# limanling/clip-event

Measured on AMD Instinct MI355X. Metric: image-text pairs/sec/GPU, ViT-B/32 224px x 77-tok, global-batch contrastive, higher is better.
Workload: dtype bf16; 1 GPU; ViT-B/32 224px x 77-tok, bf16 operands, per-GPU batch 256, K=1, InfoNCE only, full train step (fwd+bwd+clip_grad_norm+Adam), random-init weights; global_batch=256, parallelism=dp1, captions=SOT + U[8,75] random ids + EOT, zero-padded to 77 (SURVEY 8(d) c2), text_rows=live tokens SOT..EOT only: 54.8% of B*77 rows (identical results, see DESIGN.md), fresh_captions_every_step=True, alignment=False, cu_hog=0, nt_pgrid=256, full=False

## Files before the change

### clip_event_amd/csrc/attention.hip

```cpp
#include <map>
#include <mutex>

#include <type_traits>

#include "common.hpp"
#include "../../include/clip_event_hip.h"

namespace {

constexpr int HD = 64;
constexpr int ROW = 160;

typedef __attribute__((address_space(3))) s16x4 lds_s16x4;
typedef __attribute__((ext_vector_type(8))) short s16x8;

__device__ __forceinline__ bf16x8 tr_pair(const char* p0, const char* p1) {
    s16x4 lo = __builtin_amdgcn_ds_read_tr16_b64_v4i16((lds_s16x4*)p0);
    s16x4 hi = __builtin_amdgcn_ds_read_tr16_b64_v4i16((lds_s16x4*)p1);
    s16x8 v = {lo[0], lo[1], lo[2], lo[3], hi[0], hi[1], hi[2], hi[3]};
    return __builtin_bit_cast(bf16x8, v);
}

__device__ __forceinline__ bf16x8 pack8(const f32x4& a, const f32x4& b) {
    u32x4 v = {pack_bf2(a[0], a[1]), pack_bf2(a[2], a[3]), pack_bf2(b[0], b[1]), pack_bf2(b[2], b[3])};
// ... 793 lines not shown
        for (int ct = 0; ct < 4; ++ct) ak[kt][ct] *= scale;
        if (jok[kt]) {
            bf16_t* krow = dbase + (long)j[kt] * lddq + D + 4 * g;
            bf16_t* vrow = dbase + (long)j[kt] * lddq + 2 * D + 4 * g;
#pragma unroll
            for (int ct = 0; ct < 4; ++ct) {
                u32x2 pk = {pack_bf2(ak[kt][ct][0], ak[kt][ct][1]), pack_bf2(ak[kt][ct][2], ak[kt][ct][3])};
                u32x2 pv = {pack_bf2(av[kt][ct][0], av[kt][ct][1]), pack_bf2(av[kt][ct][2], av[kt][ct][3])};
                *reinterpret_cast<u32x2*>(krow + ct * 16) = pk;
                *reinterpret_cast<u32x2*>(vrow + ct * 16) = pv;
            }
        }
        if (bias_grad) {
            float vk[16], vv[16];
#pragma unroll
            for (int ct = 0; ct < 4; ++ct)
#pragma unroll
                for (int r = 0; r < 4; ++r) {
                    vk[ct * 4 + r] = ak[kt][ct][r];
                    vv[ct * 4 + r] = av[kt][ct][r];
                }
            const float tk = row16_colsum(vk, li), tv = row16_colsum(vv, li);
            const int k = row16_colsum_index(li);
            atomicAdd(&csum[(k >> 2) * 16 + 4 * g + (k & 3)], tk);
            atomicAdd(&csum[64 + (k >> 2) * 16 + 4 * g + (k & 3)], tv);
        }
    }
    if (bias_grad) {
        __syncthreads();
        if (tid < 128) atomicAdd(bias_grad + (1 + (tid >> 6)) * D + h * HD + (tid & 63), csum[tid]);
    }
}

int tiles_for(int L) { return ((L + 31) / 32) * 2; }
int attn_xcd_order() {
    static const int v = getenv("CE_ATTN_XCD") ? atoi(getenv("CE_ATTN_XCD")) : 1;
    return v;
}

struct StreamScratch { float* p = nullptr; size_t cap = 0; };
std::mutex g_scratch_mu;
std::map<hipStream_t, StreamScratch> g_scratch;
float* delta_scratch(hipStream_t s, size_t floats) {
    std::lock_guard<std::mutex> lk(g_scratch_mu);
    StreamScratch& e = g_scratch[s];
    if (e.cap < floats) {
        if (e.p) hipFree(e.p);
        e.p = nullptr; e.cap = 0;
        if (hipMalloc(reinterpret_cast<void**>(&e.p), floats * sizeof(float)) != hipSuccess) return nullptr;
        e.cap = floats;
    }
    return e.p;
}

}

#define ATTN_DISPATCH(T, CALL)                 \
    switch (T) {                               \
        case 2: CALL(2); break;                \
        case 4: CALL(4); break;                \
        case 6: CALL(6); break;                \
        case 8: CALL(8); break;                \
        default: CE_CHECK_ARG(false, "attention: sequence length %d not supported", L); \
    }

extern "C" int ce_attention_fwd(const void* qkv, long ld, void* o, long ldo, float* lse, const int* cu_seqlens, int B,
// ... 61 lines not shown
        if (nk == 1)
            hipLaunchKernelGGL(attn_bwd_long_dkv_kernel<1>, grid1, dim3(256), 0, sl, (const bf16_t*)qkv, ld, (const bf16_t*)o, ldo,
                               (const bf16_t*)dout, lddo, lse, (bf16_t*)dqkv, lddq, bias_grad, delta, L, H, D, causal, 0.125f, attn_xcd_order());
        else
            hipLaunchKernelGGL(attn_bwd_long_dkv_kernel<2>, grid2, dim3(256), 0, sl, (const bf16_t*)qkv, ld, (const bf16_t*)o, ldo,
                               (const bf16_t*)dout, lddo, lse, (bf16_t*)dqkv, lddq, bias_grad, delta, L, H, D, causal, 0.125f, attn_xcd_order());
        CE_LAUNCH_CHECK();
        return 0;
    }
    const int T = tiles_for(L);
    const int Lp = T * 16;
    int nw = T;
    if (nw > 8) nw = 8;
    const size_t lds = 2 * (size_t)Lp * ROW + 2 * (size_t)Lp * (Lp * 2 + 32);
    const float scale = 0.125f;
    hipStream_t s = (hipStream_t)stream;
    CeProfScope prof(CE_PROF_ATTN_BWD, 10.0 * B * H * (double)L * L * HD, 2.0 * (double)B * L * (8.0 * D), s);
#define CALL(TT)                                                                                                   \
    do {                                                                                                           \
        static std::once_flag attr;                                                                                \
        std::call_once(attr, [] {                                                                                  \
            hipFuncSetAttribute(reinterpret_cast<const void*>(attn_bwd_kernel<TT>),                                \
                                hipFuncAttributeMaxDynamicSharedMemorySize, 160 * 1024);                           \
        });                                                                                                        \
        hipLaunchKernelGGL(attn_bwd_kernel<TT>, dim3(B * H), dim3(64 * nw), lds, s, (const bf16_t*)qkv, ld,        \
                           (const bf16_t*)o, ldo, (const bf16_t*)dout, lddo, lse, (bf16_t*)dqkv, lddq, bias_grad, cu_seqlens, L, \
                           H, D, causal, scale);                                                                           \
    } while (0)
    ATTN_DISPATCH(T, CALL);
#undef CALL
    CE_LAUNCH_CHECK();
    return 0;
}
```

### clip_event_amd/csrc/gemm.hip

```cpp
#include <stdlib.h>

#include <map>
#include <mutex>
#include <type_traits>

#include "common.hpp"
#include "nt_plan.hpp"
#include "../../include/clip_event_hip.h"

#ifndef CE_DIAG_TN3
#define CE_DIAG_TN3 0
#endif

namespace {

constexpr int NT_BM = 128, NT_BN = 128, NT_BK = 64;
constexpr int NT_STAGE_BYTES = (NT_BM + NT_BN) * NT_BK * 2;
constexpr int NT_LDS_BYTES = 2 * NT_STAGE_BYTES;

#include "gemm_common.hpp"

template <int EPI>
__global__ __launch_bounds__(256, 2) void gemm_nt_kernel(NTArgs p) {
    extern __shared__ __attribute__((aligned(16))) char smem[];
// ... 1364 lines not shown
            const char* st = smem + cur * T2_STAGE_BYTES;
#pragma unroll
            for (int s = 0; s < 4; ++s) {
                bf16x8 pf[2], qf[2];
#pragma unroll
                for (int t = 0; t < 2; ++t) {
                    pf[t] = tr_frag2(st + offP[t] + s * 16 * 256);
                    qf[t] = tr_frag2(st + offQ[t] + s * 16 * 256);
                }
#pragma unroll
                for (int nt = 0; nt < 2; ++nt)
#pragma unroll
                    for (int kt = 0; kt < 2; ++kt)
                        acc[nt][kt] = __builtin_amdgcn_mfma_f32_32x32x16_bf16(pf[nt], qf[kt], acc[nt][kt], 0, 0, 0);
            }
            asm volatile("s_waitcnt vmcnt(0)" ::: "memory");
            __syncthreads();
        }

        const int ek = k0 + wk * 64 + (lane & 31);
        const int en = n0 + wn * 64 + 4 * (lane >> 5);
        constexpr bool sole = false;
#pragma unroll
        for (int nt = 0; nt < 2; ++nt)
#pragma unroll
            for (int kt = 0; kt < 2; ++kt) {
                const int k = ek + kt * 32;
                if (k >= p.Kk) continue;
#pragma unroll
                for (int r = 0; r < 16; ++r) {
                    const int n = en + nt * 32 + (r & 3) + 8 * (r >> 2);
                    if (n < p.Nn) {
                        float* o = p.out + (long)n * p.ldo + k;
                        if (sole) *o += acc[nt][kt][r];
                        else atomicAdd(o, acc[nt][kt][r]);
                    }
                }
            }
    }
}

template <int T3_ROWS, int T3_STAGES>
__global__ __launch_bounds__(1024, 4) void gemm_tn3_kernel(TNGroup grp) {
    constexpr int T3_IMG_BYTES = T3_ROWS * 256;
    constexpr int T3_STAGE_BYTES = 4 * T3_IMG_BYTES;
    constexpr int KSTEPS = T3_ROWS / 16;
    constexpr int DPW = T3_ROWS / 16;
    extern __shared__ __attribute__((aligned(16))) char smem[];
    const int tid = threadIdx.x;
    const int lane = tid & 63;
    const int wave = __builtin_amdgcn_readfirstlane(tid >> 6);
    const int wn = wave >> 2, wk = wave & 3;

    const int m_tiles = (grp.M + TN_BM - 1) / TN_BM;
    const int mps = grp.m_per_split / TN_BM;
    const int s_r = lane >> 4;
    const int s_chunk = (lane & 15) ^ (s_r << 2);
    const int g = lane >> 4, li = lane & 15;
    const int t_row = 8 * (g >> 1) + (li >> 2);
    const int t_sw = (li >> 2) << 2;
    const int t_cb = 2 * (g & 1) + ((li & 3) >> 1);
    int offP[2], offQ[2];
#pragma unroll
    for (int t = 0; t < 2; ++t) {
        offP[t] = (wn >> 1) * T3_IMG_BYTES + t_row * 256 + ((((wn & 1) * 8 + t * 4 + t_cb) ^ t_sw) << 4) + (li & 1) * 8;
        offQ[t] = (2 + (wk >> 1)) * T3_IMG_BYTES + t_row * 256 + ((((wk & 1) * 8 + t * 4 + t_cb) ^ t_sw) << 4) + (li & 1) * 8;
    }
// ... 586 lines not shown
            const long tail = wgs - (rounds - 1) * 256;
            return rounds * (ce_div_up(m_tiles, sp) * 1.7 + 3.0) + tail * (sp == 1 ? 0.105 : 0.20);
        };
        int sp = 1;
        if (splits > 0) sp = splits;
        else if (force_splits > 0) sp = force_splits;
        else {
            double best = cost(1);
            for (int c = 2; c <= 16 && c <= m_tiles && (long)tiles3 * c <= 256; ++c)
                if (cost(c) < best) { best = cost(c); sp = c; }
        }
        if (sp > m_tiles) sp = m_tiles;
        if (sp < 1) sp = 1;
        g.m_per_split = ce_div_up(m_tiles, sp) * TN_BM;
        g.splits = ce_div_up(M, g.m_per_split);
        g.overwrite = (overwrite && g.splits == 1) ? 1 : 0;
        if (overwrite && !g.overwrite && zero_outputs() != 0) return -5;
        static int depth = getenv("CE_TN3_DEPTH") ? atoi(getenv("CE_TN3_DEPTH")) : 3;
        g.depth = depth < 1 ? 1 : (depth > 3 ? 3 : depth);
        CeProfScope prof(CE_PROF_GEMM_TN, flops, bytes, s);
        static int rows48 = getenv("CE_TN3_ROWS") ? atoi(getenv("CE_TN3_ROWS")) != 32 : 1;
        static int lw = getenv("CE_TN3_LW") ? atoi(getenv("CE_TN3_LW")) : 1;
        if (lw && rows48)
            hipLaunchKernelGGL((gemm_tn3lw_kernel<48, 3>), dim3((unsigned)(tiles3 * g.splits)), dim3(768), 3 * 48 * 1024, s, g);
        else if (lw)
            hipLaunchKernelGGL((gemm_tn3lw_kernel<32, 4>), dim3((unsigned)(tiles3 * g.splits)), dim3(768), 4 * 32 * 1024, s, g);
        else if (rows48)
            hipLaunchKernelGGL((gemm_tn3_kernel<48, 3>), dim3((unsigned)(tiles3 * g.splits)), dim3(1024), 3 * 48 * 1024, s, g);
        else
            hipLaunchKernelGGL((gemm_tn3_kernel<32, 4>), dim3((unsigned)(tiles3 * g.splits)), dim3(1024), 4 * 32 * 1024, s, g);
        CE_LAUNCH_CHECK();
        return 0;
    }
    if (overwrite && zero_outputs() != 0) return -5;
    if (splits <= 0) splits = 512 / tiles;
    if (splits > m_tiles) splits = m_tiles;
    if (splits < 1) splits = 1;
    g.m_per_split = ce_div_up(m_tiles, splits) * TN_BM;
    g.splits = ce_div_up(M, g.m_per_split);
    CeProfScope prof(CE_PROF_GEMM_TN2, flops, bytes, s);
    hipLaunchKernelGGL(gemm_tn2_kernel, dim3((unsigned)(tiles * g.splits)), dim3(256), T2_LDS_BYTES, s, g);
    CE_LAUNCH_CHECK();
    return 0;
}

extern "C" int ce_probe_mfma(int shape, const void* a_frags, const void* b_frags, float* out, void* stream) {
    if (shape == 16)
        hipLaunchKernelGGL(probe_mfma16_kernel, dim3(1), dim3(64), 0, (hipStream_t)stream, (const bf16x8*)a_frags,
                           (const bf16x8*)b_frags, (f32x4*)out);
    else if (shape == 32)
        hipLaunchKernelGGL(probe_mfma32_kernel, dim3(1), dim3(64), 0, (hipStream_t)stream, (const bf16x8*)a_frags,
                           (const bf16x8*)b_frags, (f32x16*)out);
    else
        CE_CHECK_ARG(false, "ce_probe_mfma: shape must be 16 or 32");
    CE_LAUNCH_CHECK();
    return 0;
}

extern "C" int ce_probe_tr16(const void* image, int n_elems, const int* byte_off, void* out, void* stream) {
    CE_CHECK_ARG(n_elems > 0 && n_elems <= 16384, "ce_probe_tr16: image must hold 1..16384 elements");
    hipLaunchKernelGGL(probe_tr16_kernel, dim3(1), dim3(64), n_elems * 2, (hipStream_t)stream, (const uint16_t*)image,
                       n_elems, byte_off, (s16x4*)out);
    CE_LAUNCH_CHECK();
    return 0;
}
```

### clip_event_amd/csrc/tower.cpp

```cpp
#include <hip/hip_runtime.h>
#include <stdlib.h>

#include <map>
#include <mutex>

#include "common.hpp"
#include "../../include/clip_event_hip.h"

namespace {

constexpr int WG_MAX_BLOCKS = 8;
constexpr int WG_SETS = WG_MAX_BLOCKS + 1;
constexpr int LNP_RING = 8;

struct Carver {
    char* base;
    size_t off = 0;
    explicit Carver(void* b) : base(reinterpret_cast<char*>(b)) {}
    template <typename T>
    T* take(size_t n) {
        off = (off + 255) & ~size_t(255);
        T* p = base ? reinterpret_cast<T*>(base + off) : nullptr;
        off += n * sizeof(T);
        return p;
// ... 115 lines not shown

int linear(bool use8, const Layout& L, const void*& q8_of, const void* A, long lda, const void* W, const void* W8, const float* S8, int M,
           int N, int K, int epi, const float* bias, const void* resid, long ldr, void* out, long ldo, void* out2,
           long ldo2, const void* aux, long ldaux, void* stream) {
    if (use8 && W8 && S8 && K % 128 == 0 && K <= 4096) {
        if (q8_of != A || lda != K) TRY(ce_quant_rows_fp8(A, lda, L.q8, K, L.q8s, M, K, stream));
        q8_of = nullptr;
        return ce_gemm_nt_fp8(L.q8, K, L.q8s, W8, K, S8, M, N, K, epi, bias, resid, ldr, out, ldo, out2, ldo2, aux, ldaux,
                              stream);
    }
    return ce_gemm_nt(A, lda, W, K, M, N, K, epi, bias, resid, ldr, out, ldo, out2, ldo2, aux, ldaux, stream);
}

int forward_run(const ce_tower_desc* d, int batch, int rows, const int* cu_seqlens, const void* x0, Layout& L, void* x_out,
                const int* sel_rows, bool infer, void* stream) {
    const int M = rows, w = d->width;
    const bool f8 = (d->fp8 & 1) != 0;
    const int ST = d->stream16 ? CE_T_F16 : CE_T_F32;
    const int EPI_RESID = d->stream16 ? CE_EPI_BIAS_RESID_F16 : CE_EPI_BIAS_RESID_F32;
    const int EPI_FC = infer ? CE_EPI_BIAS_QGELU_BF16 : CE_EPI_BIAS_GELU;
    const long esz = d->stream16 ? 2 : 4;
    const void* x = x0;
    const void* q8_of = nullptr;
    const bool lnq = f8 && w % 128 == 0 && w <= 4096;
    for (int l = 0; l < d->layers; ++l) {
        const ce_block_params& p = d->blocks[l];
        BlockStash& s = L.blk[l];
        void* xo = (l + 1 < d->layers) ? s.x_out : x_out;
        TRY(ce_layernorm_fwd_q8(x, ST, w, nullptr, p.ln1_w, p.ln1_b, s.h1, CE_T_BF16, w, s.mean1, s.rstd1, M, w, 1e-5f,
                                lnq ? L.q8 : nullptr, w, L.q8s, stream));
        if (lnq) q8_of = s.h1;
        TRY(linear(f8, L, q8_of, s.h1, w, p.w_qkv, p.w8_qkv, p.s8_qkv, M, 3 * w, w, CE_EPI_BIAS_BF16, p.b_qkv, nullptr, 0, s.qkv, 3 * w, nullptr, 0,
                       nullptr, 0, stream));
        TRY(ce_attention_fwd(s.qkv, 3 * w, s.o, w, s.lse, cu_seqlens, batch, d->tokens, d->heads, d->causal, stream));
        if (sel_rows && l + 1 == d->layers) {
            const int Bn = batch;
            TRY(ce_copy_rows(s.o, w * 2L, sel_rows, L.os, w * 2L, nullptr, Bn, w * 2, stream));
            TRY(ce_copy_rows(x, w * esz, sel_rows, L.xs_in, w * esz, nullptr, Bn, (int)(w * esz), stream));
            TRY(linear(f8, L, q8_of, L.os, w, p.w_out, p.w8_out, p.s8_out, Bn, w, w, EPI_RESID, p.b_out, L.xs_in, w, L.xs_mid, w, nullptr,
                           0, nullptr, 0, stream));
            TRY(ce_layernorm_fwd_t(L.xs_mid, ST, w, nullptr, p.ln2_w, p.ln2_b, L.h2s, CE_T_BF16, w, L.means, L.rstds, Bn, w, 1e-5f, stream));
            TRY(linear(f8, L, q8_of, L.h2s, w, p.w_fc, p.w8_fc, p.s8_fc, Bn, 4 * w, w, EPI_FC, p.b_fc, nullptr, 0, infer ? L.gs : L.as, 4 * w,
                           infer ? nullptr : L.gs, infer ? 0 : 4 * w, nullptr, 0, stream));
            TRY(linear(f8, L, q8_of, L.gs, 4 * w, p.w_proj, p.w8_proj, p.s8_proj, Bn, w, 4 * w, EPI_RESID, p.b_proj, L.xs_mid, w, x_out, w,
                           nullptr, 0, nullptr, 0, stream));
            break;
        }
        TRY(linear(f8, L, q8_of, s.o, w, p.w_out, p.w8_out, p.s8_out, M, w, w, EPI_RESID, p.b_out, x, w, s.x_mid, w, nullptr, 0, nullptr,
                       0, stream));
        TRY(ce_layernorm_fwd_q8(s.x_mid, ST, w, nullptr, p.ln2_w, p.ln2_b, s.h2, CE_T_BF16, w, s.mean2, s.rstd2, M, w, 1e-5f,
                                lnq ? L.q8 : nullptr, w, L.q8s, stream));
        if (lnq) q8_of = s.h2;
        TRY(linear(f8, L, q8_of, s.h2, w, p.w_fc, p.w8_fc, p.s8_fc, M, 4 * w, w, EPI_FC, p.b_fc, nullptr, 0, infer ? s.g : s.a, 4 * w,
                       infer ? nullptr : s.g, infer ? 0 : 4 * w, nullptr, 0, stream));
        TRY(linear(f8, L, q8_of, s.g, 4 * w, p.w_proj, p.w8_proj, p.s8_proj, M, w, 4 * w, EPI_RESID, p.b_proj, s.x_mid, w, xo, w,
                       nullptr, 0, nullptr, 0, stream));
        x = xo;
    }
    return 0;
}

}

extern "C" size_t ce_tower_workspace_bytes(const ce_tower_desc* d, int batch) {
    if (check_desc(d, batch) != 0) return 0;
    Layout L;
    carve(d, batch, (size_t)batch * d->tokens, nullptr, L);
    return L.bytes;
}

// ... 104 lines not shown
    } pend;
    auto queue = [&](const void* P, long ldp, const void* Q, long ldq, int Nn, int Kk, float* out, long ldo) {
        const int i = pend.count++;
        pend.P[i] = P; pend.ldp[i] = ldp; pend.Q[i] = Q; pend.ldq[i] = ldq;
        pend.Nn[i] = Nn; pend.Kk[i] = Kk; pend.out[i] = out; pend.ldo[i] = ldo;
    };
    auto flush = [&]() -> int {
        if (pend.count == 0) return 0;
        const int rc = ce_gemm_tn_grouped_ex(pend.count, pend.P, pend.ldp, pend.Q, pend.ldq, M, pend.Nn, pend.Kk, pend.out,
                                             pend.ldo, 0, d->wgrad_overwrite, stream);
        pend.count = 0;
        pend.blocks = 0;
        return rc;
    };
    int top = layer_hi;
    if (layer_hi < last) {
    } else if (sel_rows) {
        CE_CHECK_ARG(dx_sel, "ce_tower_backward: pruned mode needs dx_sel");
        const int l = top, Bn = batch, q = l % WG_SETS;
        const ce_block_params& p = d->blocks[l];
        BlockStash& s = L.blk[l];
        const void* x_in = (l == 0) ? x0 : L.blk[l - 1].x_out;
        TRY(ce_cast_bf16(dx_sel, L.dxbs, (long)Bn * w, stream));
        TRY(linear(b8, L, q8_of, L.dxbs, w, p.wt_proj, p.wt8_proj, p.st8_proj, Bn, 4 * w, w, CE_EPI_GELUGRAD_BF16, nullptr, nullptr, 0, L.das, 4 * w, nullptr,
                       0, L.as, 4 * w, stream));
        TRY(ce_colsum_bf16(L.dxbs, w, p.g_b_proj, Bn, w, stream));
        TRY(linear(b8, L, q8_of, L.das, 4 * w, p.wt_fc, p.wt8_fc, p.st8_fc, Bn, w, 4 * w, CE_EPI_BF16, nullptr, nullptr, 0, L.dhs, w, nullptr, 0,
                       nullptr, 0, stream));
        TRY(ce_colsum_bf16(L.das, 4 * w, p.g_b_fc, Bn, 4 * w, stream));
        TRY(ce_layernorm_bwd_t(L.dhs, CE_T_BF16, w, L.xs_mid, ST, w, nullptr, L.means, L.rstds, p.ln2_w, dx_sel, CE_T_F32, L.dxs_mid,
                               ST, w, L.dxb2s, w, p.g_ln2_w, p.g_ln2_b, p.g_b_out, GS, Bn, w, stream));
        TRY(linear(b8, L, q8_of, L.dxb2s, w, p.wt_out, p.wt8_out, p.st8_out, Bn, w, w, CE_EPI_BF16, nullptr, nullptr, 0, L.dos, w, nullptr, 0, nullptr, 0,
                       stream));
        TRY(ce_scatter_rows_zero(L.dos, w * 2L, L.d_o, w * 2L, sel_rows, Bn, M, w * 2, stream));
        TRY(ce_attention_bwd(s.qkv, 3 * w, s.o, w, L.d_o, w, s.lse, L.dqkv[q], 3 * w, p.g_b_qkv, cu_seqlens, batch, d->tokens, d->heads,
                             d->causal, stream));
        {
            const void* P[3] = {L.dxbs, L.das, L.dxb2s};
            const long ldp[3] = {w, 4L * w, w};
            const void* Q[3] = {L.gs, L.h2s, L.os};
            const long ldq[3] = {4L * w, w, w};
            const int Nn[3] = {w, 4 * w, w};
            const int Kk[3] = {4 * w, w, w};
            float* out[3] = {p.g_w_proj, p.g_w_fc, p.g_w_out};
            const long ldo[3] = {4L * w, w, w};
            TRY(ce_gemm_tn_grouped_ex(3, P, ldp, Q, ldq, Bn, Nn, Kk, out, ldo, 0, d->wgrad_overwrite, stream));
        }
        queue(L.dqkv[q], 3L * w, s.h1, w, 3 * w, w, p.g_w_qkv, w);
        TRY(linear(b8, L, q8_of, L.dqkv[q], 3 * w, p.wt_qkv, p.wt8_qkv, p.st8_qkv, M, w, 3 * w, CE_EPI_BF16, nullptr, nullptr, 0, L.dh, w, nullptr, 0,
                       nullptr, 0, stream));
        TRY(ce_scatter_rows_zero(L.dxs_mid, w * esz, dx, w * esz, sel_rows, Bn, M, (int)(w * esz), stream));
        TRY(ce_layernorm_bwd_t(L.dh, CE_T_BF16, w, x_in, ST, w, nullptr, s.mean1, s.rstd1, p.ln1_w, dx, ST, dx, ST, w,
                               L.dxb[(l + WG_SETS - 1) % WG_SETS], w, p.g_ln1_w, p.g_ln1_b,
                               (l > 0) ? d->blocks[l - 1].g_b_proj : nullptr, GS, M, w, stream));
        top = l - 1;
    } else {
        if (d->stream16) TRY(ce_cast_scaled(dx, ST, L.dxb[top % WG_SETS], CE_T_BF16, GS, 1, (long)M * w, stream));
        else TRY(ce_cast_bf16(reinterpret_cast<const float*>(dx), L.dxb[top % WG_SETS], (long)M * w, stream));
    }
    plan_cuts(top, layer_lo, pend.count > 0 ? ((w % 256 == 0 && M >= 2048) ? 3L * (w / 256) * (w / 256)
                                                                              : 3L * ((w + 127) / 128) * ((w + 127) / 128)) : 0);
    for (int l = top; l >= layer_lo; --l) {
        const ce_block_params& p = d->blocks[l];
        BlockStash& s = L.blk[l];
        const int q = l % WG_SETS;
        bf16_t *dxb_a = L.dxb[q], *dxb_b = L.dxb2[q], *da = L.da[q], *dqkv = L.dqkv[q];
        const void* x_in = (l == 0) ? x0 : L.blk[l - 1].x_out;
        TRY(linear(b8, L, q8_of, dxb_a, w, p.wt_proj, p.wt8_proj, p.st8_proj, M, 4 * w, w, CE_EPI_GELUGRAD_BF16, nullptr, nullptr, 0, da, 4 * w, p.g_b_fc,
                       4 * w, s.a, 4 * w, stream));
// ... 27 lines not shown
```

### clip_event_amd/ops.py

```python
from __future__ import annotations

from ctypes import c_float, c_int, c_long, c_void_p
from typing import Optional

import torch

from . import _lib as L
from ._lib import check, lib, ptr, stream


def _rows(t: torch.Tensor) -> int:
    return t.shape[0]


def gemm_nt(a: torch.Tensor, b: torch.Tensor, epilogue: int, *, bias=None, resid=None, out=None, out2=None,
            aux=None, M: Optional[int] = None) -> torch.Tensor:
    assert a.dtype == torch.bfloat16 and b.dtype == torch.bfloat16 and a.is_cuda and b.is_cuda
    M = a.shape[0] if M is None else M
    K = a.shape[1]
    N = b.shape[0]
    assert b.shape[1] == K
    f32_out = epilogue in (L.EPI_F32, L.EPI_BIAS_F32, L.EPI_BIAS_RESID_F32)
    if epilogue == L.EPI_BIAS_RESID_F16:
        assert resid is not None and resid.dtype == torch.float16
# ... 61 lines not shown
def layernorm_bwd_t(dy, x, mean, rstd, w, dw, db, dx_out, *, gscale=None, rows=None, dx_in=None, dxb=None, dxsum=None):
    M, D = dy.shape
    check(lib().ce_layernorm_bwd_t(ptr(dy), c_int(_TYPE[dy.dtype]), c_long(dy.stride(0)), ptr(x), c_int(_TYPE[x.dtype]),
                                   c_long(x.stride(0)), ptr(rows), ptr(mean), ptr(rstd), ptr(w), ptr(dx_in),
                                   c_int(_TYPE[dx_in.dtype] if dx_in is not None else L.T_F32), ptr(dx_out),
                                   c_int(_TYPE[dx_out.dtype]), c_long(dx_out.stride(0)), ptr(dxb),
                                   c_long(dxb.stride(0) if dxb is not None else 0), ptr(dw), ptr(db), ptr(dxsum),
                                   ptr(gscale), c_int(M), c_int(D), stream()), "ce_layernorm_bwd_t")
    return dx_out


def grad_scale(x: torch.Tensor, target: float = 1024.0) -> torch.Tensor:
    assert x.dtype == torch.float32 and x.is_contiguous()
    buf = torch.empty(257, device=x.device, dtype=torch.float32)
    check(lib().ce_grad_scale(ptr(x), c_long(x.numel()), c_float(target), c_void_p(buf.data_ptr() + 4), ptr(buf), stream()),
          "ce_grad_scale")
    return buf[:1]


def cast_scaled(x: torch.Tensor, dtype, scale: torch.Tensor, divide: bool = False):
    y = torch.empty_like(x, dtype=dtype)
    check(lib().ce_cast_scaled(ptr(x), c_int(_TYPE[x.dtype]), ptr(y), c_int(_TYPE[dtype]), ptr(scale), c_int(1 if divide else 0),
                               c_long(x.numel()), stream()), "ce_cast_scaled")
    return y


def cast_t(x: torch.Tensor, dtype, mul: float = 1.0):
    y = torch.empty_like(x, dtype=dtype)
    check(lib().ce_cast_t(ptr(x), c_int(_TYPE[x.dtype]), ptr(y), c_int(_TYPE[dtype]), c_float(mul), c_long(x.numel()), stream()),
          "ce_cast_t")
    return y


def attention_fwd(qkv: torch.Tensor, B: int, L: int, H: int, causal: bool, cu_seqlens=None):
    assert qkv.dtype == torch.bfloat16
    o = torch.empty(qkv.shape[0], H * 64, device=qkv.device, dtype=torch.bfloat16)
    lse = torch.empty(B * H * L, device=qkv.device, dtype=torch.float32)
    check(lib().ce_attention_fwd(ptr(qkv), c_long(qkv.stride(0)), ptr(o), c_long(o.stride(0)), ptr(lse),
                                 ptr(cu_seqlens), c_int(B), c_int(L), c_int(H), c_int(1 if causal else 0), stream()),
          "ce_attention_fwd")
    return o, lse


def attention_bwd(qkv, o, dout, lse, B: int, L: int, H: int, causal: bool, bias_grad=None, cu_seqlens=None):
    dqkv = torch.empty_like(qkv)
    check(lib().ce_attention_bwd(ptr(qkv), c_long(qkv.stride(0)), ptr(o), c_long(o.stride(0)), ptr(dout),
                                 c_long(dout.stride(0)), ptr(lse), ptr(dqkv), c_long(dqkv.stride(0)), ptr(bias_grad),
                                 ptr(cu_seqlens), c_int(B), c_int(L), c_int(H), c_int(1 if causal else 0), stream()),
          "ce_attention_bwd")
    return dqkv


def probe_mfma(shape: int, a_frags: torch.Tensor, b_frags: torch.Tensor) -> torch.Tensor:
    out = torch.empty(64, 4 if shape == 16 else 16, device=a_frags.device, dtype=torch.float32)
    check(lib().ce_probe_mfma(c_int(shape), ptr(a_frags), ptr(b_frags), ptr(out), stream()), "ce_probe_mfma")
    return out


def probe_tr16(image: torch.Tensor, byte_off: torch.Tensor) -> torch.Tensor:
    out = torch.empty(64, 4, device=image.device, dtype=torch.int16)
    check(lib().ce_probe_tr16(ptr(image), c_int(image.numel()), ptr(byte_off), ptr(out), stream()), "ce_probe_tr16")
    return out


def quant_rows_fp8(x: torch.Tensor):
    assert x.dtype == torch.bfloat16 and x.is_cuda and x.stride(1) == 1
    M, K = x.shape
    q = torch.empty(M, K, dtype=torch.uint8, device=x.device)
    scale = torch.empty(M, dtype=torch.float32, device=x.device)
    check(lib().ce_quant_rows_fp8(ptr(x), c_long(x.stride(0)), ptr(q), c_long(K), ptr(scale), c_int(M), c_int(K), stream()),
          "ce_quant_rows_fp8")
    return q, scale


def gemm_nt_fp8(a8, sa, b8, sb, epilogue: int, *, bias=None, resid=None, aux=None, colsum=None):
    M, K = a8.shape
    N = b8.shape[0]
    f32_out = epilogue == L.EPI_BIAS_RESID_F32
# ... 56 lines not shown
```

### include/clip_event_hip.h

```cpp
#ifndef CLIP_EVENT_HIP_H
#define CLIP_EVENT_HIP_H

#include <stddef.h>
#include <stdint.h>

#ifdef __cplusplus
extern "C" {
#endif

const char* ce_last_error(void);
int ce_version(void);

enum {
    CE_EPI_BF16 = 0,
    CE_EPI_F32 = 1,
    CE_EPI_BIAS_BF16 = 2,
    CE_EPI_BIAS_F32 = 3,
    CE_EPI_BIAS_RESID_F32 = 4,
    CE_EPI_BIAS_GELU = 5,
    CE_EPI_GELUGRAD_BF16 = 6,
    CE_EPI_BIAS_RESID_F16 = 7,
    CE_EPI_BIAS_QGELU_BF16 = 8
};

// ... 46 lines not shown
int ce_layernorm_bwd(const void* dy, long lddy, int dy_f32, const float* x, long ldx, const int* rows,
                     const float* mean, const float* rstd, const float* w, const float* dx_in, float* dx_out,
                     long lddx, void* dxb, long lddxb, float* dw, float* db, float* dxsum, int M, int D,
                     void* stream);
int ce_layernorm_bwd_t(const void* dy, int dy_type, long lddy, const void* x, int x_type, long ldx, const int* rows,
                       const float* mean, const float* rstd, const float* w, const void* dx_in, int dxin_type,
                       void* dx_out, int dx_type, long lddx, void* dxb, long lddxb, float* dw, float* db, float* dxsum,
                       const float* gscale, int M, int D, void* stream);

int ce_layernorm_bwd_q8(const void* dy, int dy_type, long lddy, const void* x, int x_type, long ldx, const int* rows,
                        const float* mean, const float* rstd, const float* w, const void* dx_in, int dxin_type,
                        void* dx_out, int dx_type, long lddx, void* dxb, long lddxb, float* dw, float* db, float* dxsum,
                        const float* gscale, int M, int D, void* q8, long ldq, float* qscale, void* stream);

int ce_layernorm_bwd_blocks(int M, int D);
int ce_layernorm_bwd_partials(const void* dy, int dy_type, long lddy, const void* x, int x_type, long ldx, const int* rows,
                              const float* mean, const float* rstd, const float* w, const void* dx_in, int dxin_type,
                              void* dx_out, int dx_type, long lddx, void* dxb, long lddxb, int want_dxsum,
                              const float* gscale, int M, int D, void* q8, long ldq, float* qscale, float* partials,
                              void* stream);
#define CE_LN_FOLD_MAX 64
typedef struct ce_ln_fold_job {
    const float* partials;
    float *dw, *db, *dxsum;
    int blocks, D;
} ce_ln_fold_job;
int ce_layernorm_fold(const ce_ln_fold_job* jobs , int njobs, void* stream);

int ce_attention_fwd(const void* qkv, long ld, void* o, long ldo, float* lse, const int* cu_seqlens, int B, int L,
                     int H, int causal, void* stream);
int ce_attention_bwd(const void* qkv, long ld, const void* o, long ldo, const void* dout, long lddo,
                     const float* lse, void* dqkv, long lddq, float* bias_grad, const int* cu_seqlens, int B, int L,
                     int H, int causal, void* stream);

int ce_im2col(const float* image, void* patches, int B, int resolution, int patch, int k_padded, void* stream);
int ce_vision_assemble(const float* patch_out, const float* cls, const float* pos, float* x0, int B, int tokens,
                       int D, void* stream);
int ce_vision_assemble_bwd(const float* dx0, void* dpatch, int B, int tokens, int D, void* stream);
int ce_token_embed(const int64_t* ids, const int* src_rows, const float* table, const float* pos, float* x0, long rows,
                   int tokens, int D, int vocab, void* stream);
int ce_token_embed_t(const int64_t* ids, const int* src_rows, const float* table, const float* pos, void* x0, int x0_type,
                     long rows, int tokens, int D, int vocab, void* stream);
int ce_token_embed_bwd(const int64_t* ids, const int* src_rows, const float* dx0, float* dtable, long rows, int D,
                       int vocab, void* stream);
int ce_pos_embed_bwd_packed(const float* dx0, const int* cu_seqlens, float* dpos, int n, int tokens, int D,
                            void* stream);
int ce_batch_reduce(const float* x, float* out, int B, long slab, long n, int accumulate, void* stream);
int ce_colsum_bf16(const void* x, long ld, float* out, int M, int N, void* stream);
int ce_cast_transpose(const float* w, void* w16, long ld16, void* w16t, long ld16t, int R, int C, void* stream);
int ce_cast_bf16(const float* x, void* y, long n, void* stream);
int ce_cast_t(const void* x, int src_type, void* y, int dst_type, float mul, long n, void* stream);
int ce_cast_scaled(const void* x, int src_type, void* y, int dst_type, const float* scale, int divide, long n, void* stream);
#define CE_GRAD_SCALE_SCRATCH 256
int ce_grad_scale(const float* x, long n, float target, float* scratch, float* scale, void* stream);
int ce_stream16_set_counters(unsigned int* device_counters);
int ce_add_cols(const float* src, long lds, float* dst, long ldd, int rows, int cols, void* stream);
int ce_copy_rows(const void* src, long src_stride_bytes, const int* src_rows, void* dst, long dst_stride_bytes,
                 const int* dst_rows, int n, int row_bytes, void* stream);
int ce_scatter_rows_zero(const void* src, long src_stride_bytes, void* dst, long dst_stride_bytes, const int* dst_rows, int n,
                         int M, int row_bytes, void* stream);
int ce_eot_rows(const int64_t* ids, int* rows, long n, int tokens, void* stream);

typedef struct {
    const unsigned char* src;
    long pitch;
    int x0, y0, w, h;
// ... 155 lines not shown
```

Before: 21010 pairs/s (whole job).

## Compute last-layer attention only for selected pooled rows in fwd and bwd

In the final transformer layer only the pooled row (CLS or EOT) feeds the output, so new single-query attention kernels compute forward output and LSE just for that row per sequence and head. The backward computes dQ for that row plus dK/dV for all keys directly, and zeroes the other dQ rows. This avoids the full L×L flash-attention work and the copy-rows/scatter-zero steps. The TN2 GEMM also gains an overwrite mode when there is a single split, skipping a zeroing pass. The price is a scalar, non-MFMA path limited to L≤128 with atomics for the bias gradient.

```diff
diff --git a/clip_event_amd/csrc/attention.hip b/clip_event_amd/csrc/attention.hip
--- a/clip_event_amd/csrc/attention.hip
+++ b/clip_event_amd/csrc/attention.hip
@@ -849,6 +849,175 @@
     }
 }
 
+constexpr int SEL_WAVES = 4;
+
+__device__ __forceinline__ float bf_round(float x) { return bf_lo(pack_bf2(x, 0.f)); }
+__device__ __forceinline__ float dot8(const u32x4& a, const u32x4& b) {
+    float s = 0.f;
+#pragma unroll
+    for (int e = 0; e < 4; ++e) s += bf_lo(a[e]) * bf_lo(b[e]) + bf_hi(a[e]) * bf_hi(b[e]);
+    return s;
+}
+__device__ __forceinline__ float sum_row_lanes(float v) {
+    v += __shfl_xor(v, 1, 64);
+    v += __shfl_xor(v, 2, 64);
+    v += __shfl_xor(v, 4, 64);
+    return v;
+}
+__device__ __forceinline__ float sum_row_groups(float v) {
+    v += __shfl_xor(v, 8, 64);
+    v += __shfl_xor(v, 16, 64);
+    v += __shfl_xor(v, 32, 64);
+    return v;
+}
+__device__ __forceinline__ u32x4 pack_chunk(const float (&v)[8]) {
+    return u32x4{pack_bf2(v[0], v[1]), pack_bf2(v[2], v[3]), pack_bf2(v[4], v[5]), pack_bf2(v[6], v[7])};
+}
+
+struct SelCoords { int b, h, L, i; long row0; };
+__device__ __forceinline__ bool sel_coords(const int* cu, const int* sel, int Lmax, int H, SelCoords& c) {
+    const int wave = __builtin_amdgcn_readfirstlane(threadIdx.x >> 6);
+    const int hg = (H + SEL_WAVES - 1) / SEL_WAVES;
+    c.b = blockIdx.x / hg;
+    c.h = (blockIdx.x - c.b * hg) * SEL_WAVES + wave;
+    if (c.h >= H) return false;
+    c.row0 = cu ? (long)cu[c.b] : (long)c.b * Lmax;
+    c.L = cu ? min(cu[c.b + 1] - cu[c.b], Lmax) : Lmax;
+    if (c.L <= 0) return false;
+    c.i = min(max((int)((long)sel[c.b] - c.row0), 0), c.L - 1);
+    return true;
+}
+
+template <int NIT>
+__device__ __forceinline__ void sel_load_kv(const bf16_t* srcK, const bf16_t* srcV, long ld, int n, int lane, u32x4 (&kk)[NIT], u32x4 (&vv)[NIT]) {
+    const uint32_t span = (uint32_t)(((long)n - 1) * ld * 2 + HD * 2);
+    const __amdgpu_buffer_rsrc_t rK = make_rsrc(srcK, span), rV = make_rsrc(srcV, span);
+#pragma unroll
+    for (int it = 0; it < NIT; ++it) {
+        const int j = it * 8 + (lane >> 3);
+        const uint32_t off = j < n ? (uint32_t)(j * ld * 2 + (lane & 7) * 16) : 0x80000000u;
+        kk[it] = __builtin_amdgcn_raw_buffer_load_b128(rK, off, 0, 0);
+        vv[it] = __builtin_amdgcn_raw_buffer_load_b128(rV, off, 0, 0);
+    }
+}
+
+template <int NIT>
+__global__ __launch_bounds__(64 * SEL_WAVES) void attn_fwd_sel_kernel(const bf16_t* __restrict__ qkv, long ld, bf16_t* __restrict__ o_sel,
+                                                                      long ldo, float* __restrict__ lse, const int* __restrict__ cu,
+                                                                      const int* __restrict__ sel, int Lmax, int H, int D, int causal,
+                                                                      float scale) {
+    SelCoords sc;
+    if (!sel_coords(cu, sel, Lmax, H, sc)) return;
+    const int lane = threadIdx.x & 63, r8 = lane >> 3, c = lane & 7;
+    const int n = causal ? sc.i + 1 : sc.L;
+    const bf16_t* base = qkv + sc.row0 * ld + sc.h * HD;
+    const u32x4 q = *reinterpret_cast<const u32x4*>(base + (long)sc.i * ld + c * 8);
+    u32x4 kk[NIT], vv[NIT];
+    sel_load_kv<NIT>(base + D, base + 2 * D, ld, n, lane, kk, vv);
+    float s[NIT], mx = -INFINITY;
+#pragma unroll
+    for (int it = 0; it < NIT; ++it) {
+        const float d = sum_row_lanes(dot8(kk[it], q));
+        s[it] = (it * 8 + r8 < n) ? d * scale : -INFINITY;
+        mx = fmaxf(mx, s[it]);
+    }
+    mx = fmaxf(mx, __shfl_xor(mx, 8, 64));
+    mx = fmaxf(mx, __shfl_xor(mx, 16, 64));
+    mx = fmaxf(mx, __shfl_xor(mx, 32, 64));
+    float sum = 0.f, acc[8] = {0.f, 0.f, 0.f, 0.f, 0.f, 0.f, 0.f, 0.f};
+#pragma unroll
+    for (int it = 0; it < NIT; ++it) {
+        const float p = __expf(s[it] - mx);
+        sum += p;
+        const float pb = bf_round(p);
+#pragma unroll
+        for (int e = 0; e < 4; ++e) {
+            acc[2 * e] += pb * bf_lo(vv[it][e]);
+            acc[2 * e + 1] += pb * bf_hi(vv[it][e]);
+        }
+    }
+    sum = sum_row_groups(sum);
+    const float inv = 1.0f / sum;
+#pragma unroll
+    for (int e = 0; e < 8; ++e) acc[e] = sum_row_groups(acc[e]) * inv;
+    if (r8 == 0) *reinterpret_cast<u32x4*>(o_sel + (long)sc.b * ldo + sc.h * HD + c * 8) = pack_chunk(acc);
+    if (lane == 0) lse[((long)sc.b * H + sc.h) * Lmax + sc.i] = mx + __logf(sum);
+}
+
+template <int NIT>
+__global__ __launch_bounds__(64 * SEL_WAVES) void attn_bwd_sel_kernel(const bf16_t* __restrict__ qkv, long ld, const bf16_t* __restrict__ o_sel,
+                                                                      long ldo, const bf16_t* __restrict__ do_sel, long lddo,
+                                                                      const float* __restrict__ lse, bf16_t* __restrict__ dqkv, long lddq,
+                                                                      float* __restrict__ bias_grad, const int* __restrict__ cu,
+                                                                      const int* __restrict__ sel, int Lmax, int H, int D, int causal,
+                                                                      float scale) {
+    SelCoords sc;
+    if (!sel_coords(cu, sel, Lmax, H, sc)) return;
+    const int lane = threadIdx.x & 63, r8 = lane >> 3, c = lane & 7;
+    const int n = causal ? sc.i + 1 : sc.L;
+    const bf16_t* base = qkv + sc.row0 * ld + sc.h * HD;
+    const u32x4 q = *reinterpret_cast<const u32x4*>(base + (long)sc.i * ld + c * 8);
+    const u32x4 dO = *reinterpret_cast<const u32x4*>(do_sel + (long)sc.b * lddo + sc.h * HD + c * 8);
+    const u32x4 O = *reinterpret_cast<const u32x4*>(o_sel + (long)sc.b * ldo + sc.h * HD + c * 8);
+    const float lsei = lse[((long)sc.b * H + sc.h) * Lmax + sc.i];
+    const bf16_t qcol = bias_grad ? base[(long)sc.i * ld + lane] : (bf16_t)0;
+    const bf16_t dcol = bias_grad ? do_sel[(long)sc.b * lddo + sc.h * HD + lane] : (bf16_t)0;
+    u32x4 kk[NIT], vv[NIT];
+    sel_load_kv<NIT>(base + D, base + 2 * D, ld, n, lane, kk, vv);
+    const float dl = sum_row_lanes(dot8(dO, O));
+    float qf[8], df[8];
+#pragma unroll
+    for (int e = 0; e < 4; ++e) {
+        qf[2 * e] = bf_lo(q[e]); qf[2 * e + 1] = bf_hi(q[e]);
+        df[2 * e] = bf_lo(dO[e]); df[2 * e + 1] = bf_hi(dO[e]);
+    }
+    bf16_t* dbase = dqkv + sc.row0 * lddq + sc.h * HD + c * 8;
+    float dq[8] = {0.f, 0.f, 0.f, 0.f, 0.f, 0.f, 0.f, 0.f}, sds = 0.f, sp = 0.f;
+#pragma unroll
+    for (int it = 0; it < NIT; ++it) {
+        const int j = it * 8 + r8;
+        const float sd = sum_row_lanes(dot8(kk[it], q)), dp = sum_row_lanes(dot8(vv[it], dO));
+        const float p = j < n ? __expf(sd * scale - lsei) : 0.f;
+        const float pb = bf_round(p), dsb = bf_round(p * (dp - dl) * scale);
+        sds += dsb;
+        sp += pb;
+        float dk[8], dv[8];
+#pragma unroll
+        for (int e = 0; e < 4; ++e) {
+            dq[2 * e] += dsb * bf_lo(kk[it][e]);
+            dq[2 * e + 1] += dsb * bf_hi(kk[it][e]);
+        }
+#pragma unroll
+        for (int e = 0; e < 8; ++e) {
+            dk[e] = dsb * qf[e];
+            dv[e] = pb * df[e];
+        }
+        if (j < sc.L) {
+            bf16_t* row = dbase + (long)j * lddq;
+            if (j != sc.i) *reinterpret_cast<u32x4*>(row) = u32x4{0u, 0u, 0u, 0u};
+            *reinterpret_cast<u32x4*>(row + D) = pack_chunk(dk);
+            *reinterpret_cast<u32x4*>(row + 2 * D) = pack_chunk(dv);
+        }
+    }
+#pragma unroll
+    for (int e = 0; e < 8; ++e) dq[e] = sum_row_groups(dq[e]);
+    if (r8 == 0) *reinterpret_cast<u32x4*>(dbase + (long)sc.i * lddq) = pack_chunk(dq);
+    if (bias_grad) {
+        sds = sum_row_groups(sds);
+        sp = sum_row_groups(sp);
+        float dqc = 0.f;
+#pragma unroll
+        for (int e = 0; e < 8; ++e) {
+            const float t = __shfl(dq[e], lane >> 3, 64);
+            if ((lane & 7) == e) dqc = t;
+        }
+        float* dst = bias_grad + sc.h * HD + lane;
+        atomicAdd(dst, dqc);
+        atomicAdd(dst + D, sds * __uint_as_float((uint32_t)qcol << 16));
+        atomicAdd(dst + 2 * D, sp * __uint_as_float((uint32_t)dcol << 16));
+    }
+}
+
 int tiles_for(int L) { return ((L + 31) / 32) * 2; }
 int attn_xcd_order() {
     static const int v = getenv("CE_ATTN_XCD") ? atoi(getenv("CE_ATTN_XCD")) : 1;
@@ -976,3 +1145,43 @@
     CE_LAUNCH_CHECK();
     return 0;
 }
+
+extern "C" int ce_attention_fwd_sel(const void* qkv, long ld, void* o_sel, long ldo, float* lse, const int* cu_seqlens,
+                                    const int* sel_rows, int B, int L, int H, int causal, void* stream) {
+    CE_CHECK_ARG(B > 0 && L > 0 && H > 0, "ce_attention_fwd_sel: empty problem");
+    CE_CHECK_ARG(L <= 128, "ce_attention_fwd_sel: sequences of at most 128 tokens (got %d)", L);
+    CE_CHECK_ARG(sel_rows && qkv && o_sel && lse, "ce_attention_fwd_sel: null buffer");
+    CE_CHECK_ARG(ld % 8 == 0 && ldo % 8 == 0 && (long)L * ld < (1L << 29), "ce_attention_fwd_sel: bad leading dimension");
+    const int D = H * HD, T = tiles_for(L);
+    hipStream_t s = (hipStream_t)stream;
+    CeProfScope prof(CE_PROF_ATTN_FWD, 4.0 * B * H * (double)L * HD, 2.0 * (double)B * L * (2.0 * D), s);
+    const dim3 grid(B * ((H + SEL_WAVES - 1) / SEL_WAVES)), block(64 * SEL_WAVES);
+#define CALL(TT)                                                                                                              \
+    hipLaunchKernelGGL(attn_fwd_sel_kernel<2 * TT>, grid, block, 0, s, (const bf16_t*)qkv, ld, (bf16_t*)o_sel, ldo, lse, cu_seqlens, \
+                       sel_rows, L, H, D, causal, 0.125f)
+    ATTN_DISPATCH(T, CALL);
+#undef CALL
+    CE_LAUNCH_CHECK();
+    return 0;
+}
+
+extern "C" int ce_attention_bwd_sel(const void* qkv, long ld, const void* o_sel, long ldo, const void* do_sel, long lddo,
+                                    const float* lse, void* dqkv, long lddq, float* bias_grad, const int* cu_seqlens,
+                                    const int* sel_rows, int B, int L, int H, int causal, void* stream) {
+    CE_CHECK_ARG(B > 0 && L > 0 && H > 0, "ce_attention_bwd_sel: empty problem");
+    CE_CHECK_ARG(L <= 128, "ce_attention_bwd_sel: sequences of at most 128 tokens (got %d)", L);
+    CE_CHECK_ARG(sel_rows && qkv && o_sel && do_sel && lse && dqkv, "ce_attention_bwd_sel: null buffer");
+    CE_CHECK_ARG(ld % 8 == 0 && ldo % 8 == 0 && lddo % 8 == 0 && lddq % 8 == 0 && (long)L * ld < (1L << 29),
+                 "ce_attention_bwd_sel: bad leading dimension");
+    const int D = H * HD, T = tiles_for(L);
+    hipStream_t s = (hipStream_t)stream;
+    CeProfScope prof(CE_PROF_ATTN_BWD, 10.0 * B * H * (double)L * HD, 2.0 * (double)B * L * (5.0 * D), s);
+    const dim3 grid(B * ((H + SEL_WAVES - 1) / SEL_WAVES)), block(64 * SEL_WAVES);
+#define CALL(TT)                                                                                                                  \
+    hipLaunchKernelGGL(attn_bwd_sel_kernel<2 * TT>, grid, block, 0, s, (const bf16_t*)qkv, ld, (const bf16_t*)o_sel, ldo,        \
+                       (const bf16_t*)do_sel, lddo, lse, (bf16_t*)dqkv, lddq, bias_grad, cu_seqlens, sel_rows, L, H, D, causal, 0.125f)
+    ATTN_DISPATCH(T, CALL);
+#undef CALL
+    CE_LAUNCH_CHECK();
+    return 0;
+}
diff --git a/clip_event_amd/csrc/gemm.hip b/clip_event_amd/csrc/gemm.hip
--- a/clip_event_amd/csrc/gemm.hip
+++ b/clip_event_amd/csrc/gemm.hip
@@ -1420,7 +1420,8 @@
                     const int n = en + nt * 32 + (r & 3) + 8 * (r >> 2);
                     if (n < p.Nn) {
                         float* o = p.out + (long)n * p.ldo + k;
-                        if (sole) *o += acc[nt][kt][r];
+                        if (grp.overwrite) *o = acc[nt][kt][r];
+                        else if (sole) *o += acc[nt][kt][r];
                         else atomicAdd(o, acc[nt][kt][r]);
                     }
                 }
@@ -2073,12 +2074,13 @@
         CE_LAUNCH_CHECK();
         return 0;
     }
-    if (overwrite && zero_outputs() != 0) return -5;
     if (splits <= 0) splits = 512 / tiles;
     if (splits > m_tiles) splits = m_tiles;
     if (splits < 1) splits = 1;
     g.m_per_split = ce_div_up(m_tiles, splits) * TN_BM;
     g.splits = ce_div_up(M, g.m_per_split);
+    g.overwrite = (overwrite && g.splits == 1) ? 1 : 0;
+    if (overwrite && !g.overwrite && zero_outputs() != 0) return -5;
     CeProfScope prof(CE_PROF_GEMM_TN2, flops, bytes, s);
     hipLaunchKernelGGL(gemm_tn2_kernel, dim3((unsigned)(tiles * g.splits)), dim3(256), T2_LDS_BYTES, s, g);
     CE_LAUNCH_CHECK();
diff --git a/clip_event_amd/csrc/tower.cpp b/clip_event_amd/csrc/tower.cpp
--- a/clip_event_amd/csrc/tower.cpp
+++ b/clip_event_amd/csrc/tower.cpp
@@ -171,10 +171,13 @@
         if (lnq) q8_of = s.h1;
         TRY(linear(f8, L, q8_of, s.h1, w, p.w_qkv, p.w8_qkv, p.s8_qkv, M, 3 * w, w, CE_EPI_BIAS_BF16, p.b_qkv, nullptr, 0, s.qkv, 3 * w, nullptr, 0,
                        nullptr, 0, stream));
-        TRY(ce_attention_fwd(s.qkv, 3 * w, s.o, w, s.lse, cu_seqlens, batch, d->tokens, d->heads, d->causal, stream));
-        if (sel_rows && l + 1 == d->layers) {
+        const bool pruned = sel_rows && l + 1 == d->layers;
+        const bool sel_attn = pruned && d->tokens <= 128;
+        if (sel_attn) TRY(ce_attention_fwd_sel(s.qkv, 3 * w, L.os, w, s.lse, cu_seqlens, sel_rows, batch, d->tokens, d->heads, d->causal, stream));
+        else TRY(ce_attention_fwd(s.qkv, 3 * w, s.o, w, s.lse, cu_seqlens, batch, d->tokens, d->heads, d->causal, stream));
+        if (pruned) {
             const int Bn = batch;
-            TRY(ce_copy_rows(s.o, w * 2L, sel_rows, L.os, w * 2L, nullptr, Bn, w * 2, stream));
+            if (!sel_attn) TRY(ce_copy_rows(s.o, w * 2L, sel_rows, L.os, w * 2L, nullptr, Bn, w * 2, stream));
             TRY(ce_copy_rows(x, w * esz, sel_rows, L.xs_in, w * esz, nullptr, Bn, (int)(w * esz), stream));
             TRY(linear(f8, L, q8_of, L.os, w, p.w_out, p.w8_out, p.s8_out, Bn, w, w, EPI_RESID, p.b_out, L.xs_in, w, L.xs_mid, w, nullptr,
                            0, nullptr, 0, stream));
@@ -345,9 +348,14 @@
                                ST, w, L.dxb2s, w, p.g_ln2_w, p.g_ln2_b, p.g_b_out, GS, Bn, w, stream));
         TRY(linear(b8, L, q8_of, L.dxb2s, w, p.wt_out, p.wt8_out, p.st8_out, Bn, w, w, CE_EPI_BF16, nullptr, nullptr, 0, L.dos, w, nullptr, 0, nullptr, 0,
                        stream));
-        TRY(ce_scatter_rows_zero(L.dos, w * 2L, L.d_o, w * 2L, sel_rows, Bn, M, w * 2, stream));
-        TRY(ce_attention_bwd(s.qkv, 3 * w, s.o, w, L.d_o, w, s.lse, L.dqkv[q], 3 * w, p.g_b_qkv, cu_seqlens, batch, d->tokens, d->heads,
-                             d->causal, stream));
+        if (d->tokens <= 128) {
+            TRY(ce_attention_bwd_sel(s.qkv, 3 * w, L.os, w, L.dos, w, s.lse, L.dqkv[q], 3 * w, p.g_b_qkv, cu_seqlens, sel_rows, batch,
+                                     d->tokens, d->heads, d->causal, stream));
+        } else {
+            TRY(ce_scatter_rows_zero(L.dos, w * 2L, L.d_o, w * 2L, sel_rows, Bn, M, w * 2, stream));
+            TRY(ce_attention_bwd(s.qkv, 3 * w, s.o, w, L.d_o, w, s.lse, L.dqkv[q], 3 * w, p.g_b_qkv, cu_seqlens, batch, d->tokens, d->heads,
+                                 d->causal, stream));
+        }
         {
             const void* P[3] = {L.dxbs, L.das, L.dxb2s};
             const long ldp[3] = {w, 4L * w, w};
diff --git a/clip_event_amd/ops.py b/clip_event_amd/ops.py
--- a/clip_event_amd/ops.py
+++ b/clip_event_amd/ops.py
@@ -117,18 +117,30 @@
     return y
 
 
-def attention_fwd(qkv: torch.Tensor, B: int, L: int, H: int, causal: bool, cu_seqlens=None):
+def attention_fwd(qkv: torch.Tensor, B: int, L: int, H: int, causal: bool, cu_seqlens=None, *, sel_rows=None):
     assert qkv.dtype == torch.bfloat16
+    lse = torch.empty(B * H * L, device=qkv.device, dtype=torch.float32)
+    if sel_rows is not None:
+        o = torch.empty(B, H * 64, device=qkv.device, dtype=torch.bfloat16)
+        check(lib().ce_attention_fwd_sel(ptr(qkv), c_long(qkv.stride(0)), ptr(o), c_long(o.stride(0)), ptr(lse),
+                                         ptr(cu_seqlens), ptr(sel_rows), c_int(B), c_int(L), c_int(H), c_int(1 if causal else 0),
+                                         stream()), "ce_attention_fwd_sel")
+        return o, lse
     o = torch.empty(qkv.shape[0], H * 64, device=qkv.device, dtype=torch.bfloat16)
-    lse = torch.empty(B * H * L, device=qkv.device, dtype=torch.float32)
     check(lib().ce_attention_fwd(ptr(qkv), c_long(qkv.stride(0)), ptr(o), c_long(o.stride(0)), ptr(lse),
                                  ptr(cu_seqlens), c_int(B), c_int(L), c_int(H), c_int(1 if causal else 0), stream()),
           "ce_attention_fwd")
     return o, lse
 
 
-def attention_bwd(qkv, o, dout, lse, B: int, L: int, H: int, causal: bool, bias_grad=None, cu_seqlens=None):
+def attention_bwd(qkv, o, dout, lse, B: int, L: int, H: int, causal: bool, bias_grad=None, cu_seqlens=None, *, sel_rows=None):
     dqkv = torch.empty_like(qkv)
+    if sel_rows is not None:
+        check(lib().ce_attention_bwd_sel(ptr(qkv), c_long(qkv.stride(0)), ptr(o), c_long(o.stride(0)), ptr(dout),
+                                         c_long(dout.stride(0)), ptr(lse), ptr(dqkv), c_long(dqkv.stride(0)), ptr(bias_grad),
+                                         ptr(cu_seqlens), ptr(sel_rows), c_int(B), c_int(L), c_int(H), c_int(1 if causal else 0),
+                                         stream()), "ce_attention_bwd_sel")
+        return dqkv
     check(lib().ce_attention_bwd(ptr(qkv), c_long(qkv.stride(0)), ptr(o), c_long(o.stride(0)), ptr(dout),
                                  c_long(dout.stride(0)), ptr(lse), ptr(dqkv), c_long(dqkv.stride(0)), ptr(bias_grad),
                                  ptr(cu_seqlens), c_int(B), c_int(L), c_int(H), c_int(1 if causal else 0), stream()),
diff --git a/include/clip_event_hip.h b/include/clip_event_hip.h
--- a/include/clip_event_hip.h
+++ b/include/clip_event_hip.h
@@ -102,6 +102,11 @@
 int ce_attention_bwd(const void* qkv, long ld, const void* o, long ldo, const void* dout, long lddo,
                      const float* lse, void* dqkv, long lddq, float* bias_grad, const int* cu_seqlens, int B, int L,
                      int H, int causal, void* stream);
+int ce_attention_fwd_sel(const void* qkv, long ld, void* o_sel, long ldo, float* lse, const int* cu_seqlens,
+                         const int* sel_rows, int B, int L, int H, int causal, void* stream);
+int ce_attention_bwd_sel(const void* qkv, long ld, const void* o_sel, long ldo, const void* do_sel, long lddo,
+                         const float* lse, void* dqkv, long lddq, float* bias_grad, const int* cu_seqlens,
+                         const int* sel_rows, int B, int L, int H, int causal, void* stream);
 
 int ce_im2col(const float* image, void* patches, int B, int resolution, int patch, int k_padded, void* stream);
 int ce_vision_assemble(const float* patch_out, const float* cls, const float* pos, float* x0, int B, int tokens,
```

Result: no change. 21140 pairs/s (whole job), median of 6 (+0.6%).
